# bartelvdh/Navtex

Hardware: AMD Instinct MI355X
Metric: IQ Msamples/s through FIR->FSK->bitsync (higher is better)
Workload: dtype f64

## Files before the change

### navtex_amd/csrc/nvx_demod.hip

```cpp
#include <hip/hip_runtime.h>
#include <stdint.h>
#include <stdlib.h>

#include "nvx_tables.h"
#include "nvx_atan2.h"
#include "nvx_fsm.h"
#include "nvx_kernels.h"

enum { DS_Y3 = 0, DS_DPHI = 8, DS_S = 16, DS_C = 24, DS_COUNT = 24 + 567 };
enum { DI_SYNCED = 0, DI_SYNC_OFF, DI_NEXT_SYNC_OFF, DI_PHASE, DI_PREV_OFFSET, DI_COUNT };
static_assert(DI_COUNT == NVX_DEMOD_INTS && DS_COUNT == NVX_DEMOD_DOUBLES && DI_PREV_OFFSET == NVX_DI_PREV_OFFSET &&
              DI_PHASE == NVX_DI_PHASE, "state layout");

#ifndef NVX_FRONT_THREADS
#define NVX_FRONT_THREADS 128
#endif
#ifndef DTL
#define DTL NVX_FRONT_TILE
static_assert(DTL % 9 == 0, "a tile is a whole number of bit periods");
#endif
#define FRONT_SLIDE ((567 + NVX_FRONT_THREADS - 1) / NVX_FRONT_THREADS)
#define G_DAB 8
#define G_CB 574
#define G_CSA 582

__device__ __forceinline__ double2 y3_at(const double2 *y3, const double *hist, int t)
{
    if (t >= 0) return y3[t];
    double2 r; r.x = hist[2 * (4 + t)]; r.y = hist[2 * (4 + t) + 1];
    return r;
}

__device__ __forceinline__ double front_dphi(double2 s, double2 p)
{
    const double prodReal = s.x * p.x + s.y * p.y;
    const double prodImg  = s.y * p.x - s.x * p.y;
    return nvx_atan2(prodImg, prodReal);
}
__device__ __forceinline__ void front_energies(double2 w0, double2 w1, double2 w2, double2 w3, double2 w4,
                                               float &Brot, float &Yrot)
{
    float BR = 0.0f, BI = 0.0f, YR = 0.0f, YI = 0.0f;
#pragma unroll
    for (int i = 0; i < 5; i++) {
        const double2 w = i == 0 ? w0 : i == 1 ? w1 : i == 2 ? w2 : i == 3 ? w3 : w4;
        const float fR = NVX_BF_R[i], fI = NVX_BF_I[i];
        const double sampleR = w.x, sampleI = w.y;
        YR = (float)((double)YR + ((double)((float)sampleR * fR) - sampleI * (double)fI));
        YI = (float)((double)YI + ((double)((float)sampleR * fI) + sampleI * (double)fR));
        BR = (float)((double)BR + ((double)((float)sampleR * fR) + sampleI * (double)fI));
        BI = (float)((double)BI + ((double)((float)(-sampleR) * fI) + sampleI * (double)fR));
    }
    Brot = BR * BR + BI * BI;
    Yrot = YR * YR + YI * YI;
}
__device__ __forceinline__ unsigned char front_decision(double2 w0, double2 w1, double2 w2, double2 w3, double2 w4, float &hi, float &lo)
{
    float Brot, Yrot;
    front_energies(w0, w1, w2, w3, w4, Brot, Yrot);
    const bool b = Brot > Yrot;
    hi = b ? Brot : Yrot; lo = b ? Yrot : Brot;
    return b ? 1 : 0;
}

struct FrontSig { double power, dphi_b, dphi2_b, dphi_y, dphi2_y, hi, lo; unsigned nb, pad; };
__device__ __forceinline__ void front_sig_init(FrontSig &s)
{
    s.power = s.dphi_b = s.dphi2_b = s.dphi_y = s.dphi2_y = s.hi = s.lo = 0.0; s.nb = s.pad = 0;
}
__device__ __forceinline__ void front_sig_add(FrontSig &s, double2 y, double ds, unsigned char d, float hi, float lo)
{
    s.power += y.x * y.x + y.y * y.y;
    const double b = d ? ds : 0.0, m = d ? 0.0 : ds;
    s.dphi_b += b; s.dphi2_b += b * b; s.dphi_y += m; s.dphi2_y += m * m;
    s.hi += (double)hi; s.lo += (double)lo; s.nb += d;
}
__device__ __forceinline__ double front_wave_sum(double v)
{
#pragma unroll
    for (int o = 32; o >= 1; o >>= 1) v += __shfl_xor(v, o);
    return v;
}
__device__ __forceinline__ unsigned front_wave_sum(unsigned v)
{
#pragma unroll
    for (int o = 32; o >= 1; o >>= 1) v += __shfl_xor(v, o);
    return v;
}
__device__ __forceinline__ void front_sig_publish(FrontSig s, unsigned n, FrontSig *s_w, nvx_sig_rec *rec, int tid)
{
    s.power = front_wave_sum(s.power); s.dphi_b = front_wave_sum(s.dphi_b); s.dphi2_b = front_wave_sum(s.dphi2_b);
    s.dphi_y = front_wave_sum(s.dphi_y); s.dphi2_y = front_wave_sum(s.dphi2_y); s.hi = front_wave_sum(s.hi); s.lo = front_wave_sum(s.lo);
    s.nb = front_wave_sum(s.nb);
    if ((tid & 63) == 0) s_w[tid >> 6] = s;
    __syncthreads();
    if (tid == 0) {
        FrontSig t = s_w[0];
#pragma unroll
        for (int w = 1; w < NVX_FRONT_THREADS / 64; w++) {
            const FrontSig &u = s_w[w];
            t.power += u.power; t.dphi_b += u.dphi_b; t.dphi2_b += u.dphi2_b; t.dphi_y += u.dphi_y; t.dphi2_y += u.dphi2_y;
            t.hi += u.hi; t.lo += u.lo; t.nb += u.nb;
        }
        nvx_sig_rec r;
        r.sum_power = t.power; r.sum_dphi_b = t.dphi_b; r.sum_dphi2_b = t.dphi2_b; r.sum_dphi_y = t.dphi_y; r.sum_dphi2_y = t.dphi2_y;
        r.sum_mf_hi = t.hi; r.sum_mf_lo = t.lo; r.samples = n; r.b_samples = t.nb;
        *rec = r;
    }
}
__device__ __forceinline__ double front_corr(const double *dp)
{
    double temp = 0.0;
#pragma unroll
    for (int i = 0; i < 9; i++) temp += (double)NVX_CORR_MASK[i] * dp[i];
    return __builtin_fabs(temp);
}
__device__ __forceinline__ double front_class_sum(const double *cnow, unsigned u)
{
    const unsigned c = u % 9u;
    const int d0 = (int)((u + 566u - c) % 567u);
    const int jw = d0 / 9;
    const double *run1 = cnow - d0;
    const double *run2 = run1 - 567;
    double temp = 0.0;
#pragma unroll
    for (int j = 0; j < 63; j++) temp += (j <= jw ? run1 : run2)[9 * j];
    return temp;
}
struct FrontTies { unsigned near, evals; float minm; };
__device__ __forceinline__ FrontTies front_ties_init() { FrontTies t; t.near = 0; t.evals = 0; t.minm = __uint_as_float(0x7f800000u); return t; }
__device__ __forceinline__ unsigned short front_word(const unsigned char *d9, const double *sv, bool evaluate, FrontTies &ties)
{
    unsigned w = 0;
#pragma unroll
    for (int k = 0; k < 9; k++) w |= (unsigned)d9[k] << k;
    unsigned max_index = 15;
    if (evaluate) {
        double temp_max = -1.0, runner_up = -1.0;
        max_index = 0;
#pragma unroll
        for (int i = 0; i < 9; i++) {
            const double v = sv[i];
            if (v > temp_max) { runner_up = temp_max; temp_max = v; max_index = i; }
            else if (v > runner_up) runner_up = v;
        }
        if (temp_max > 0.0) {
            const double margin = temp_max - runner_up;
            ties.evals++;
            if (margin < temp_max * 0x1p-40) ties.near++;
            ties.minm = fminf(ties.minm, (float)(margin / temp_max));
        }
    }
    return (unsigned short)(w | (max_index << 12));
}

struct FrontChain { int slot; unsigned long long g0; const double *st_rd; double *st_wr; int n3; };
__device__ __forceinline__ FrontChain front_chain(const nvx_demod_args &a, int chain_index)
{
    FrontChain c;
    c.slot = chain_index; c.g0 = a.g0; c.n3 = a.n3;
    int parity = 0;
    if (a.part) {
        const int per = 2 * a.per_part, e = chain_index / per;
        c.slot = a.part[e].stream * per + (chain_index - e * per);
        c.g0 = a.part[e].g0; parity = a.part[e].parity; c.n3 = a.part[e].n3;
    }
    c.st_rd = (parity ? a.dstate[1] : a.dstate[0]) + (size_t)c.slot * NVX_DEMOD_DOUBLES;
    c.st_wr = (parity ? a.dstate[0] : a.dstate[1]) + (size_t)c.slot * NVX_DEMOD_DOUBLES;
    return c;
}

__device__ __forceinline__ void front_publish_ties(const nvx_demod_args &a, const FrontTies &t, unsigned *s_near, unsigned *s_evals, unsigned *s_minm, int tid)
{
    if (t.evals) { atomicAdd(s_near, t.near); atomicAdd(s_evals, t.evals); atomicMin(s_minm, __float_as_uint(t.minm)); }
    __syncthreads();
    if (tid == 0 && *s_evals) {
        if (*s_near) atomicAdd(&a.ties->near_ties, (unsigned long long)*s_near);
        atomicAdd(&a.ties->evaluations, (unsigned long long)*s_evals);
        atomicMin(&a.ties->min_margin_bits, *s_minm);
    }
}

struct FrontWalkLds {
    double dphi[8 + DTL];
    double S[8 + DTL];
    double C[567 + DTL];
    unsigned char D[DTL];
    unsigned near, evals, minm;
    FrontSig sig[NVX_FRONT_THREADS / 64];
};
template <bool SIG>
__device__ __forceinline__ void front_sequential(const nvx_demod_args &a, int chain_index, int n_tiles_here, FrontWalkLds &lds)
{
    double *const s_dphi = lds.dphi, *const s_S = lds.S, *const s_C = lds.C;
    unsigned char *const s_D = lds.D;
    unsigned &s_near = lds.near, &s_evals = lds.evals, &s_minm = lds.minm;
    const int tid = threadIdx.x;
    const FrontChain ch = front_chain(a, chain_index);
    const int slot = ch.slot;
    if (!a.slot_active[slot]) return;
    if (tid == 0) { s_near = 0; s_evals = 0; s_minm = 0x7f800000u; }
    FrontTies ties = front_ties_init();
    constexpr bool sig_on = SIG;
    FrontSig sig;
    front_sig_init(sig);

    const double *st = ch.st_rd;
    const double2 *y3 = a.y3 + (size_t)slot * a.y3_cap + a.y3_base;
    double *dphi_out = a.dphi ? a.dphi + (size_t)slot * a.y3_cap + a.y3_base : nullptr;
    double *corr_out = a.corr ? a.corr + (size_t)slot * a.y3_cap + a.y3_base : nullptr;
    double *csum_out = a.csum ? a.csum + (size_t)slot * a.y3_cap + a.y3_base : nullptr;
    const double *hist = st + DS_Y3;
    if (tid < 8) { s_dphi[tid] = st[DS_DPHI + tid]; s_S[tid] = st[DS_S + tid]; }
    for (int i = tid; i < 567; i += NVX_FRONT_THREADS) s_C[i] = st[DS_C + i];
    __syncthreads();

    const int n3 = ch.n3;
    const int n_here = n_tiles_here > 0 ? min(n3, n_tiles_here * DTL) : n3;
    for (int ta = 0; ta < n_here; ta += DTL) {
        const int tl = min(DTL, n_here - ta);
        const int tl9 = (tl + 8) / 9;
        const unsigned long long gt = ch.g0 + (unsigned long long)ta;
        for (int L = tid; L < tl; L += NVX_FRONT_THREADS) {
            const int t = ta + L;
            const double2 w3 = y3_at(y3, hist, t - 1), w4 = y3[t];
            const double ds = front_dphi(w4, w3);
            s_dphi[8 + L] = ds;
            if (dphi_out) dphi_out[t] = ds;
            float hi, lo;
            const unsigned char d = front_decision(y3_at(y3, hist, t - 4), y3_at(y3, hist, t - 3), y3_at(y3, hist, t - 2), w3, w4, hi, lo);
            s_D[L] = d;
            if (sig_on && gt + L >= G_DAB) front_sig_add(sig, w4, ds, d, hi, lo);
        }
        if (tid < 9 * tl9 - tl) s_D[tl + tid] = 0;
        __syncthreads();
        for (int L = tid; L < tl; L += NVX_FRONT_THREADS)
            s_C[567 + L] = (gt + L >= G_DAB) ? front_corr(&s_dphi[L]) : 0.0;
        __syncthreads();
        const unsigned t_cb = (unsigned)((gt % 5103u + (5103u - G_CB % 5103u)) % 5103u);
        for (int L = tid; L < tl; L += NVX_FRONT_THREADS)
            s_S[8 + L] = (gt + L >= G_CB) ? front_class_sum(&s_C[567 + L], t_cb + (unsigned)L) : 0.0;
        __syncthreads();
        if (corr_out)
            for (int L = tid; L < tl; L += NVX_FRONT_THREADS) { corr_out[ta + L] = s_C[567 + L]; csum_out[ta + L] = s_S[8 + L]; }
        for (int M = tid; M < tl9; M += NVX_FRONT_THREADS) {
            const int L = 9 * M + (G_CSA % 9);
            a.words[(size_t)slot * (a.y3_cap / 9) + (ta / 9 + M)] = front_word(&s_D[9 * M], &s_S[L], L < tl && gt + L >= G_CSA, ties);
        }
        __syncthreads();
        double h_d = 0.0, h_s = 0.0, h_c[FRONT_SLIDE];
        if (tid < 8) { h_d = s_dphi[tl + tid]; h_s = s_S[tl + tid]; }
#pragma unroll
        for (int k = 0; k < FRONT_SLIDE; k++) { const int i = tid + NVX_FRONT_THREADS * k; h_c[k] = (i < 567) ? s_C[tl + i] : 0.0; }
        __syncthreads();
        if (tid < 8) { s_dphi[tid] = h_d; s_S[tid] = h_s; }
#pragma unroll
        for (int k = 0; k < FRONT_SLIDE; k++) { const int i = tid + NVX_FRONT_THREADS * k; if (i < 567) s_C[i] = h_c[k]; }
        __syncthreads();
    }

    front_publish_ties(a, ties, &s_near, &s_evals, &s_minm, tid);
    if (sig_on) {
        const unsigned skip = ch.g0 >= G_DAB ? 0u : (unsigned)min((unsigned long long)n_here, G_DAB - ch.g0);
        front_sig_publish(sig, (unsigned)n_here - skip, lds.sig, a.sig_part + (size_t)slot * a.sig_stride, tid);
    }
    if (n_tiles_here > 0) return;
    double *sw = ch.st_wr;
    if (tid < 4 && n3 >= 4) { const double2 l = y3[n3 - 4 + tid]; sw[DS_Y3 + 2 * tid] = l.x; sw[DS_Y3 + 2 * tid + 1] = l.y; }
    if (tid < 8) { sw[DS_DPHI + tid] = s_dphi[tid]; sw[DS_S + tid] = s_S[tid]; }
    for (int i = tid; i < 567; i += NVX_FRONT_THREADS) sw[DS_C + i] = s_C[i];
}

__global__ __launch_bounds__(NVX_FRONT_THREADS) __attribute__((amdgpu_waves_per_eu(5))) void nvx_demod_front(nvx_demod_args a)
{
    __shared__ FrontWalkLds lds;
    if (a.sig) front_sequential<true>(a, blockIdx.x, 0, lds);
    else front_sequential<false>(a, blockIdx.x, 0, lds);
}

#define FRONT_LOOKBACK 576
__global__ __launch_bounds__(NVX_FRONT_THREADS) void nvx_demod_front_head(nvx_demod_args a)
{
    __shared__ FrontWalkLds lds;
    if (a.sig) front_sequential<true>(a, blockIdx.x, 2, lds);
    else front_sequential<false>(a, blockIdx.x, 2, lds);
}
__global__ __launch_bounds__(NVX_FRONT_THREADS) void nvx_demod_front_tiles(nvx_demod_args a, int wgs_per_chain)
{
    const int chain_index = blockIdx.x / wgs_per_chain, wg = blockIdx.x - chain_index * wgs_per_chain;
    __shared__ double p_dphi[FRONT_LOOKBACK + DTL];
    __shared__ double p_C[FRONT_LOOKBACK - 8 + DTL];
    __shared__ double p_S[2 + DTL];
    __shared__ unsigned char p_D[DTL];
    __shared__ unsigned s_near, s_evals, s_minm;
    __shared__ FrontSig s_sig[NVX_FRONT_THREADS / 64];
    const int tid = threadIdx.x;
    const FrontChain ch = front_chain(a, chain_index);
    const int slot = ch.slot;
    if (!a.slot_active[slot]) return;
    if (tid == 0) { s_near = 0; s_evals = 0; s_minm = 0x7f800000u; }
    FrontTies ties = front_ties_init();
    const int ta = (wg + 2) * DTL;
    const int tl = min(DTL, a.n3 - ta);
    const double2 *y3 = a.y3 + (size_t)slot * a.y3_cap + a.y3_base;
    double *dphi_out = a.dphi ? a.dphi + (size_t)slot * a.y3_cap + a.y3_base : nullptr;
    double *corr_out = a.corr ? a.corr + (size_t)slot * a.y3_cap + a.y3_base : nullptr;
    double *csum_out = a.csum ? a.csum + (size_t)slot * a.y3_cap + a.y3_base : nullptr;
    const unsigned long long g_ta = ch.g0 + (unsigned long long)ta;
    const bool sig_on = a.sig != nullptr;
    FrontSig sig;
    front_sig_init(sig);

    for (int i = tid; i < FRONT_LOOKBACK + tl; i += NVX_FRONT_THREADS) {
        const int t = ta - FRONT_LOOKBACK + i;
        const double ds = front_dphi(y3[t], y3[t - 1]);
        p_dphi[i] = ds;
        if (i >= FRONT_LOOKBACK) {
            if (dphi_out) dphi_out[t] = ds;
            float hi, lo;
            const unsigned char d = front_decision(y3[t - 4], y3[t - 3], y3[t - 2], y3[t - 1], y3[t], hi, lo);
            p_D[i - FRONT_LOOKBACK] = d;
            if (sig_on) front_sig_add(sig, y3[t], ds, d, hi, lo);
        }
    }
    __syncthreads();
    for (int i = tid; i < FRONT_LOOKBACK - 8 + tl; i += NVX_FRONT_THREADS)
        p_C[i] = (g_ta - 568 + (unsigned long long)i >= G_DAB) ? front_corr(&p_dphi[i]) : 0.0;
    __syncthreads();
    const unsigned t_cb = (unsigned)(((g_ta - 2) % 5103u + (5103u - G_CB % 5103u)) % 5103u);
    for (int i = tid; i < 2 + tl; i += NVX_FRONT_THREADS)
        p_S[i] = (g_ta - 2 + (unsigned long long)i >= G_CB) ? front_class_sum(&p_C[566 + i], t_cb + (unsigned)i) : 0.0;
    __syncthreads();
    if (corr_out)
        for (int i = tid; i < tl; i += NVX_FRONT_THREADS) { corr_out[ta + i] = p_C[FRONT_LOOKBACK - 8 + i]; csum_out[ta + i] = p_S[2 + i]; }
    for (int M = tid; M < tl / 9; M += NVX_FRONT_THREADS)
        a.words[(size_t)slot * (a.y3_cap / 9) + (ta / 9 + M)] = front_word(&p_D[9 * M], &p_S[9 * M], g_ta + 9 * M + (G_CSA % 9) >= G_CSA, ties);
    front_publish_ties(a, ties, &s_near, &s_evals, &s_minm, tid);
    if (sig_on) front_sig_publish(sig, (unsigned)tl, s_sig, a.sig_part + (size_t)slot * a.sig_stride + 1 + wg, tid);
    if (ta + tl >= a.n3) {
        double *sw = ch.st_wr;
        if (tid < 4) { const double2 l = y3[a.n3 - 4 + tid]; sw[DS_Y3 + 2 * tid] = l.x; sw[DS_Y3 + 2 * tid + 1] = l.y; }
        if (tid < 8) { sw[DS_DPHI + tid] = p_dphi[FRONT_LOOKBACK + tl - 8 + tid]; sw[DS_S + tid] = p_S[2 + tl - 8 + tid]; }
        for (int i = tid; i < 567; i += NVX_FRONT_THREADS) sw[DS_C + i] = p_C[FRONT_LOOKBACK - 8 + tl - 567 + i];
    }
}

#ifndef NVX_SOFT_INFLIGHT
#define NVX_SOFT_INFLIGHT 2
#endif
template <bool HIST>
__device__ __forceinline__ float fsm_soft_at(const double2 *y3, const double *hist, int t)
{
    double2 w[5];
#pragma unroll
    for (int i = 0; i < 5; i++) w[i] = HIST ? y3_at(y3, hist, t - 4 + i) : y3[t - 4 + i];
    float Brot, Yrot;
    front_energies(w[0], w[1], w[2], w[3], w[4], Brot, Yrot);
    return Brot - Yrot;
}
__device__ __forceinline__ int fsm_soft_period(const double2 *y3, const double *hist, int m, unsigned p, float *row, int cap, int j)
{
    const int n = NVX_FSM_POS_N(p);
    if (n >= 1) { const float v = fsm_soft_at<true>(y3, hist, 9 * m + NVX_FSM_POS_K1(p)); if (j < cap) row[j] = v; j++; }
    if (n == 2) { const float v = fsm_soft_at<true>(y3, hist, 9 * m + NVX_FSM_POS_K2(p)); if (j < cap) row[j] = v; j++; }
    return j;
}

template <bool SOFT>
__device__ __forceinline__ void fsm_chain(const nvx_demod_args &a, const uint32_t *s_tab)
{
    int slot = blockIdx.x * 64 + threadIdx.x;
    const int nc = a.n_slots;
    int n3 = a.n3, parity = 0;
    if (a.part) {
        const int per = 2 * a.per_part, e = slot / per;
        if (e >= a.n_part) return;
        slot = a.part[e].stream * per + (slot - e * per);
        n3 = a.part[e].n3; parity = a.part[e].parity;
    }
    if (slot >= nc) return;
    if (!a.slot_active[slot]) return;
    int *si = a.state_i;
#define SI(f) si[(size_t)(f) * nc + slot]
    nvx_fsm_regs r;
    r.so = SI(DI_SYNCED) ? SI(DI_SYNC_OFF) : NVX_FSM_UNSYNCED;
    r.nso = SI(DI_NEXT_SYNC_OFF);
    r.phase1 = SI(DI_PHASE) + 1;
    r.prev_offset = SI(DI_PREV_OFFSET);

    unsigned *bits = (unsigned *)(a.bits + (size_t)slot * a.bits_cap);
    const int cap_words = a.bits_cap / 4;
    unsigned long long acc = 0;
    int nacc = 0, nwords = 0;
    const int periods = n3 / 9;
    const unsigned short *wrow = a.words + (size_t)slot * (a.y3_cap / 9);
    const uint4 *words = (const uint4 *)wrow;
    uint4 wnext = words[0];
    unsigned short *prow = SOFT ? a.soft_pos + (size_t)slot * (a.y3_cap / 9) : nullptr;

    int m0 = 0;
    for (; m0 + 8 <= periods; m0 += 8) {
        const uint4 wv = wnext;
        if (m0 + 16 <= periods) wnext = words[m0 / 8 + 1];
        const unsigned wcur[8] = { wv.x & 0xffffu, wv.x >> 16, wv.y & 0xffffu, wv.y >> 16,
                                   wv.z & 0xffffu, wv.z >> 16, wv.w & 0xffffu, wv.w >> 16 };
        unsigned pcur[8];
#pragma unroll
        for (int i = 0; i < 8; i++) {
            int n;
            const unsigned b = nvx_fsm_period_pos(s_tab, wcur[i], &r, &n, &pcur[i]);
            acc |= (unsigned long long)(b & ((1u << n) - 1u)) << nacc;
            nacc += n;
        }
        if (SOFT) {
            uint4 pv;
            pv.x = pcur[0] | pcur[1] << 16; pv.y = pcur[2] | pcur[3] << 16; pv.z = pcur[4] | pcur[5] << 16; pv.w = pcur[6] | pcur[7] << 16;
            ((uint4 *)prow)[m0 / 8] = pv;
        }
        if (nacc >= 32) {
            if (nwords < cap_words) bits[nwords] = (unsigned)acc;
            nwords++; acc >>= 32; nacc -= 32;
        }
    }
    for (; m0 < periods; m0++) {
        int n;
        unsigned pos;
        const unsigned b = nvx_fsm_period_pos(s_tab, wrow[m0], &r, &n, &pos);
        if (SOFT) prow[m0] = (unsigned short)pos;
        acc |= (unsigned long long)(b & ((1u << n) - 1u)) << nacc;
        nacc += n;
        if (nacc >= 32) { if (nwords < cap_words) bits[nwords] = (unsigned)acc; nwords++; acc >>= 32; nacc -= 32; }
    }
    const int rem = n3 - 9 * periods;
    if (rem) {
        const unsigned w = wrow[periods];
        int n;
        unsigned pos;
        const unsigned b = nvx_fsm_partial_period_pos(w, rem, &r, &n, &pos);
        if (SOFT) prow[periods] = (unsigned short)pos;
        acc |= (unsigned long long)(b & ((1u << n) - 1u)) << nacc;
        nacc += n;
        if (nacc >= 32) { if (nwords < cap_words) bits[nwords] = (unsigned)acc; nwords++; acc >>= 32; nacc -= 32; }
    }
    if (nacc > 0 && nwords < cap_words) bits[nwords] = (unsigned)acc;

    a.nbits[slot] = nwords * 32 + nacc;
    const int synced = r.so != NVX_FSM_UNSYNCED;
    SI(DI_SYNCED) = synced; SI(DI_SYNC_OFF) = synced ? r.so : 0; SI(DI_NEXT_SYNC_OFF) = r.nso;
    SI(DI_PHASE) = r.phase1 - 1; SI(DI_PREV_OFFSET) = r.prev_offset;
#undef SI
    if (SOFT) {
        const double2 *y3 = a.y3 + (size_t)slot * a.y3_cap + a.y3_base;
        const double *hist = (parity ? a.dstate[1] : a.dstate[0]) + (size_t)slot * NVX_DEMOD_DOUBLES + DS_Y3;
        float *row = a.soft + (size_t)slot * a.soft_cap;
        const int cap = a.soft_cap;
        const int whole = periods & ~7;
        int j = 0, m = 0;
        const uint4 *notes = (const uint4 *)prow;
        if (whole) {
            const uint4 pv = notes[0];
            const unsigned pcur[8] = { pv.x & 0xffffu, pv.x >> 16, pv.y & 0xffffu, pv.y >> 16,
                                       pv.z & 0xffffu, pv.z >> 16, pv.w & 0xffffu, pv.w >> 16 };
#pragma unroll
            for (int i = 0; i < 8; i++) j = fsm_soft_period(y3, hist, i, pcur[i], row, cap, j);
            m = 8;
        }
        uint4 pnext = whole > 8 ? notes[1] : uint4{ 0, 0, 0, 0 };
        for (; m < whole; m += 8) {
            const uint4 pv = pnext;
            if (m + 16 <= whole) pnext = notes[m / 8 + 1];
            const unsigned pcur[8] = { pv.x & 0xffffu, pv.x >> 16, pv.y & 0xffffu, pv.y >> 16,
                                       pv.z & 0xffffu, pv.z >> 16, pv.w & 0xffffu, pv.w >> 16 };
#pragma unroll
            for (int i = 0; i < 8; i += NVX_SOFT_INFLIGHT) {
                float v[NVX_SOFT_INFLIGHT];
#pragma unroll
                for (int u = 0; u < NVX_SOFT_INFLIGHT; u++)
                    v[u] = fsm_soft_at<false>(y3, hist, 9 * (m + i + u) + (NVX_FSM_POS_N(pcur[i + u]) ? NVX_FSM_POS_K1(pcur[i + u]) : 8));
#pragma unroll
                for (int u = 0; u < NVX_SOFT_INFLIGHT; u++) {
                    const int n = NVX_FSM_POS_N(pcur[i + u]);
                    if (n >= 1) { if (j < cap) row[j] = v[u]; j++; }
                    if (n == 2) {
                        const float v2 = fsm_soft_at<false>(y3, hist, 9 * (m + i + u) + NVX_FSM_POS_K2(pcur[i + u]));
                        if (j < cap) row[j] = v2;
                        j++;
                    }
                }
            }
        }
        for (; m < periods + (rem ? 1 : 0); m++) j = fsm_soft_period(y3, hist, m, prow[m], row, cap, j);
    }
    if (a.sig) {
        const nvx_sig_rec *p = a.sig_part + (size_t)slot * a.sig_stride;
        nvx_sig_rec s = p[0];
        for (int k = 1; k < a.sig_parts; k++) {
            const nvx_sig_rec &q = p[k];
            s.sum_power += q.sum_power; s.sum_dphi_b += q.sum_dphi_b; s.sum_dphi2_b += q.sum_dphi2_b;
            s.sum_dphi_y += q.sum_dphi_y; s.sum_dphi2_y += q.sum_dphi2_y; s.sum_mf_hi += q.sum_mf_hi; s.sum_mf_lo += q.sum_mf_lo;
            s.samples += q.samples; s.b_samples += q.b_samples;
        }
        a.sig[slot] = s;
    }
}

__global__ __launch_bounds__(64) void nvx_demod_fsm(nvx_demod_args a)
{
    __shared__ uint32_t s_tab[NVX_FSM_TABLE_ALLOC];
    {
        const uint4 *src = (const uint4 *)a.fsm_table;
        uint4 *dst = (uint4 *)s_tab;
        for (int i = threadIdx.x; i < NVX_FSM_TABLE_ALLOC / 4; i += 64) dst[i] = src[i];
    }
    __syncthreads();
    if (a.soft) fsm_chain<true>(a, s_tab);
    else fsm_chain<false>(a, s_tab);
}

extern "C" int nvx_front_tile_wgs(const nvx_demod_args *a, int request)
{
    const unsigned chains = a->part ? (unsigned)(2 * a->per_part * a->n_part) : (unsigned)a->n_slots;
    const int tiles = (a->n3 + DTL - 1) / DTL;
    const long long chain_frames = (long long)chains * (a->n3 / NVX_Y3_PER_FRAME);
    const bool parallel = tiles >= 3 && (request >= 0 ? request != 0 : chain_frames <= 2560);
    return parallel ? tiles - 2 : 0;
}

extern "C" hipError_t nvx_launch_demod_front(const nvx_demod_args *a, hipStream_t s)
{
    const unsigned chains = a->part ? (unsigned)(2 * a->per_part * a->n_part) : (unsigned)a->n_slots;
    const int wgs = a->sig_parts - 1;
    if (wgs < 0) return hipErrorInvalidValue;
    if (a->sig && 1 + wgs > a->sig_stride) return hipErrorInvalidValue;
    if (wgs) {
        hipLaunchKernelGGL(nvx_demod_front_head, dim3(chains), dim3(NVX_FRONT_THREADS), 0, s, *a);
        hipLaunchKernelGGL(nvx_demod_front_tiles, dim3(chains * (unsigned)wgs), dim3(NVX_FRONT_THREADS), 0, s, *a, wgs);
    } else {
        hipLaunchKernelGGL(nvx_demod_front, dim3(chains), dim3(NVX_FRONT_THREADS), 0, s, *a);
    }
    return hipGetLastError();
}

extern "C" hipError_t nvx_launch_demod_fsm(const nvx_demod_args *a, hipStream_t s)
{
    const int chains = a->part ? 2 * a->per_part * a->n_part : a->n_slots;
    if (a->sig_parts < 1) return hipErrorInvalidValue;
    hipLaunchKernelGGL(nvx_demod_fsm, dim3((unsigned)((chains + 63) / 64)), dim3(64), 0, s, *a);
    return hipGetLastError();
}

extern "C" __attribute__((visibility("default"))) double nvx_atan2_host(double y, double x) { return nvx_atan2(y, x); }
```

Measured before the change: 1.547 million.

## Compute class sums per 9-sample group with register accumulators split across half-blocks

Replaces the per-sample 63-term strided class sum with a per-group routine. Each thread handles a group of 9 consecutive outputs: one half of the block computes 5 of the columns and the other half computes 4, reusing the shared jw/run selection and using vectorised LDS loads with pinned accumulation order. The aim is to cut redundant index arithmetic and per-element LDS address work in the dominant front-end reduction. In exchange it reads a few elements before the C buffer, which requires the S-before-C layout assertion and an 8-element pad in the tiles kernel. It also makes the priming bounds scalar.

```diff
diff --git a/navtex_amd/csrc/nvx_demod.hip b/navtex_amd/csrc/nvx_demod.hip
--- a/navtex_amd/csrc/nvx_demod.hip
+++ b/navtex_amd/csrc/nvx_demod.hip
@@ -6,6 +6,7 @@
 #include "nvx_atan2.h"
 #include "nvx_fsm.h"
 #include "nvx_kernels.h"
+#include "nvx_device.h"
 
 enum { DS_Y3 = 0, DS_DPHI = 8, DS_S = 16, DS_C = 24, DS_COUNT = 24 + 567 };
 enum { DI_SYNCED = 0, DI_SYNC_OFF, DI_NEXT_SYNC_OFF, DI_PHASE, DI_PREV_OFFSET, DI_COUNT };
@@ -115,17 +116,55 @@
     for (int i = 0; i < 9; i++) temp += (double)NVX_CORR_MASK[i] * dp[i];
     return __builtin_fabs(temp);
 }
-__device__ __forceinline__ double front_class_sum(const double *cnow, unsigned u)
-{
-    const unsigned c = u % 9u;
-    const int d0 = (int)((u + 566u - c) % 567u);
-    const int jw = d0 / 9;
-    const double *run1 = cnow - d0;
-    const double *run2 = run1 - 567;
-    double temp = 0.0;
-#pragma unroll
-    for (int j = 0; j < 63; j++) temp += (j <= jw ? run1 : run2)[9 * j];
-    return temp;
+#ifndef FRONT_GROUP_TERMS
+#define FRONT_GROUP_TERMS 3
+#endif
+template <int C0, int NC>
+__device__ __forceinline__ void front_group_sums(const double *c_at, double *s_at, int n, int n_unprimed, unsigned u0, int lane, int n_lanes)
+{
+    const int c_first = (int)(u0 % 9u);
+    const unsigned m_first = ((u0 - (unsigned)c_first) / 9u + 62u) % 63u;
+    const int n_groups = (c_first + n + 8) / 9;
+    for (int q = lane; q < n_groups; q += n_lanes) {
+        const int e0 = 9 * q - c_first;
+        const int jw = (int)((m_first + (unsigned)q) % 63u);
+        const lds_vdouble *run1 = (const lds_vdouble *)(c_at + (e0 - (9 * jw + 8)) + C0);
+        const lds_vdouble *run2 = run1 - 567;
+        NVX_PIN_AFTER(run2);
+        double acc[NC];
+#pragma unroll
+        for (int k = 0; k < NC; k++) acc[k] = 0.0;
+#pragma unroll
+        for (int j = 0; j < 63; j++) {
+            const lds_vdouble *run = j <= jw ? run1 : run2;
+            double v[NC];
+#pragma unroll
+            for (int k = 0; k < NC; k++) v[k] = run[9 * j + k];
+#pragma unroll
+            for (int k = 0; k < NC; k++) acc[k] += v[k];
+            if (j % FRONT_GROUP_TERMS == FRONT_GROUP_TERMS - 1) {
+#pragma unroll
+                for (int k = 0; k < NC; k++) NVX_PIN_AFTER(acc[k]);
+            }
+        }
+#pragma unroll
+        for (int k = 0; k < NC; k++) {
+            const int e = e0 + C0 + k;
+            if (e >= 0 && e < n) s_at[e] = e >= n_unprimed ? acc[k] : 0.0;
+        }
+    }
+}
+static_assert((NVX_FRONT_THREADS / 2) % 64 == 0, "a class half is whole waves");
+__device__ __forceinline__ void front_class_sums(const double *c_at, double *s_at, int n, int n_unprimed, unsigned u0, int tid)
+{
+    constexpr int H = NVX_FRONT_THREADS / 2;
+    if (tid < H) front_group_sums<0, 5>(c_at, s_at, n, n_unprimed, u0, tid, H);
+    else front_group_sums<5, 4>(c_at, s_at, n, n_unprimed, u0, tid - H, H);
+}
+__device__ __forceinline__ int front_unprimed(unsigned long long g_first, unsigned long long g_at, int n)
+{
+    const long long d = (long long)g_at - (long long)g_first;
+    return d <= 0 ? 0 : d >= (long long)n ? n : (int)d;
 }
 struct FrontTies { unsigned near, evals; float minm; };
 __device__ __forceinline__ FrontTies front_ties_init() { FrontTies t; t.near = 0; t.evals = 0; t.minm = __uint_as_float(0x7f800000u); return t; }
@@ -189,6 +228,7 @@
     unsigned near, evals, minm;
     FrontSig sig[NVX_FRONT_THREADS / 64];
 };
+static_assert(offsetof(FrontWalkLds, C) == offsetof(FrontWalkLds, S) + sizeof(double) * (8 + DTL), "S lies directly in front of C");
 template <bool SIG>
 __device__ __forceinline__ void front_sequential(const nvx_demod_args &a, int chain_index, int n_tiles_here, FrontWalkLds &lds)
 {
@@ -234,12 +274,12 @@
         }
         if (tid < 9 * tl9 - tl) s_D[tl + tid] = 0;
         __syncthreads();
+        const int n_dab = front_unprimed(gt, G_DAB, tl);
         for (int L = tid; L < tl; L += NVX_FRONT_THREADS)
-            s_C[567 + L] = (gt + L >= G_DAB) ? front_corr(&s_dphi[L]) : 0.0;
+            s_C[567 + L] = (L >= n_dab) ? front_corr(&s_dphi[L]) : 0.0;
         __syncthreads();
         const unsigned t_cb = (unsigned)((gt % 5103u + (5103u - G_CB % 5103u)) % 5103u);
-        for (int L = tid; L < tl; L += NVX_FRONT_THREADS)
-            s_S[8 + L] = (gt + L >= G_CB) ? front_class_sum(&s_C[567 + L], t_cb + (unsigned)L) : 0.0;
+        front_class_sums(&s_C[567], &s_S[8], tl, front_unprimed(gt, G_CB, tl), t_cb, tid);
         __syncthreads();
         if (corr_out)
             for (int L = tid; L < tl; L += NVX_FRONT_THREADS) { corr_out[ta + L] = s_C[567 + L]; csum_out[ta + L] = s_S[8 + L]; }
@@ -289,7 +329,8 @@
 {
     const int chain_index = blockIdx.x / wgs_per_chain, wg = blockIdx.x - chain_index * wgs_per_chain;
     __shared__ double p_dphi[FRONT_LOOKBACK + DTL];
-    __shared__ double p_C[FRONT_LOOKBACK - 8 + DTL];
+    __shared__ double p_C8[8 + FRONT_LOOKBACK - 8 + DTL];
+    double *const p_C = p_C8 + 8;
     __shared__ double p_S[2 + DTL];
     __shared__ unsigned char p_D[DTL];
     __shared__ unsigned s_near, s_evals, s_minm;
@@ -328,8 +369,7 @@
         p_C[i] = (g_ta - 568 + (unsigned long long)i >= G_DAB) ? front_corr(&p_dphi[i]) : 0.0;
     __syncthreads();
     const unsigned t_cb = (unsigned)(((g_ta - 2) % 5103u + (5103u - G_CB % 5103u)) % 5103u);
-    for (int i = tid; i < 2 + tl; i += NVX_FRONT_THREADS)
-        p_S[i] = (g_ta - 2 + (unsigned long long)i >= G_CB) ? front_class_sum(&p_C[566 + i], t_cb + (unsigned)i) : 0.0;
+    front_class_sums(&p_C[566], p_S, 2 + tl, front_unprimed(g_ta - 2, G_CB, 2 + tl), t_cb, tid);
     __syncthreads();
     if (corr_out)
         for (int i = tid; i < tl; i += NVX_FRONT_THREADS) { corr_out[ta + i] = p_C[FRONT_LOOKBACK - 8 + i]; csum_out[ta + i] = p_S[2 + i]; }
```

After: 1.558 million, median of 6. No clear change (+0.7%).
